# TUMFTM/global_racetrajectory_optimization

Measured on NVIDIA H100. Metric: min-curv QPs/sec (N=1000 closed track, batched), higher is better.
Workload: dtype f64

## Files before the change

### global_racetrajectory_optimization_b200/csrc/mincurv_ipm.cu

```cuda
#include <cstdio>
#include <cstdlib>
#include "mincurv_ops.cuh"

namespace mc {

constexpr unsigned FULL = 0xffffffffu;
constexpr int IP_THREADS = 64;
constexpr int SUB = 8;
constexpr int VBP = 12;
constexpr int FROW = 34;
constexpr int HB_SLOTS = 2;
constexpr int HO_SLOTS = 2;
constexpr int LROW = 33;
#ifndef MC_LT_SLOTS
#define MC_LT_SLOTS 3
#endif
constexpr int LT_SLOTS = MC_LT_SLOTS;
constexpr int GT_SLOTS = 6 - LT_SLOTS;
constexpr int RING_UNITS = LT_SLOTS + GT_SLOTS;
constexpr int QDEPTH = 16;
constexpr int LT_UNIT_DOUBLES = SUB * LROW;
constexpr int GT_UNIT_DOUBLES = SUB * FROW;
constexpr unsigned HB_UNIT_BYTES = SUB * HB_PITCH * sizeof(double);

__device__ __forceinline__ void dmma(double (&c)[2], double a, double b) {
    asm volatile("mma.sync.aligned.m8n8k4.row.col.f64.f64.f64.f64 {%0,%1}, {%2}, {%3}, {%0,%1};\n"
                 : "+d"(c[0]), "+d"(c[1]) : "d"(a), "d"(b));
}

__device__ __forceinline__ uint32_t smem_u32(const void *p) { return (uint32_t)__cvta_generic_to_shared(p); }
__device__ __forceinline__ void mbar_init(uint64_t *bar, unsigned count) {
    asm volatile("mbarrier.init.shared::cta.b64 [%0], %1;" ::"r"(smem_u32(bar)), "r"(count) : "memory");
}
__device__ __forceinline__ void mbar_expect_tx(uint64_t *bar, unsigned bytes) {
    asm volatile("mbarrier.arrive.expect_tx.shared::cta.b64 _, [%0], %1;" ::"r"(smem_u32(bar)), "r"(bytes) : "memory");
}
__device__ __forceinline__ void mbar_arrive(uint64_t *bar) {
    asm volatile("mbarrier.arrive.shared::cta.b64 _, [%0];" ::"r"(smem_u32(bar)) : "memory");
}
#ifndef MC_WAIT_MODE
#define MC_WAIT_MODE 1
#endif
#ifndef MC_RELAXED_BACKOFF_NS
#define MC_RELAXED_BACKOFF_NS 250
#endif

__device__ __forceinline__ void mbar_wait(uint64_t *bar, unsigned parity) {
#if MC_WAIT_MODE == 0
    asm volatile("{\n .reg .pred p;\n WAIT_%=:\n mbarrier.try_wait.parity.shared::cta.b64 p, [%0], %1, 0x989680;\n"
                 " @p bra DONE_%=;\n bra WAIT_%=;\n DONE_%=:\n}" ::"r"(smem_u32(bar)), "r"(parity) : "memory");
#else
    asm volatile("{\n .reg .pred p;\n WAIT_%=:\n mbarrier.test_wait.parity.shared::cta.b64 p, [%0], %1;\n"
                 " @p bra DONE_%=;\n bra WAIT_%=;\n DONE_%=:\n}" ::"r"(smem_u32(bar)), "r"(parity) : "memory");
#endif
}
__device__ __forceinline__ void mbar_wait_relaxed(uint64_t *bar, unsigned parity) {
#ifndef MC_RELAXED_SPIN_NS
    unsigned ok = 0;
    for (;;) {
        asm volatile("{\n .reg .pred p;\n mbarrier.try_wait.parity.shared::cta.b64 p, [%1], %2, 0x989680;\n selp.u32 %0, 1, 0, p;\n}"
                     : "=r"(ok) : "r"(smem_u32(bar)), "r"(parity) : "memory");
        if (ok) break;
        __nanosleep(MC_RELAXED_BACKOFF_NS);
// ... 61 lines not shown
#define SEG_BEGIN() do { } while (0)
#define SEG(slot) do { } while (0)
#define PROF_T0(name) do { } while (0)
#define PROF_ADD(slot, t0) do { } while (0)
#define PROF_ADD1(slot, t0) do { } while (0)
#endif

__device__ __forceinline__ double fast_rcp(double d) {
    double x;
    asm("rcp.approx.ftz.f64 %0, %1;" : "=d"(x) : "d"(d));
    double e = fma(-d, x, 1.0);
    x = fma(x, e, x);
    e = fma(-d, x, 1.0);
    return fma(x, e, x);
}

struct Handoff {
    double vb[32 * VBP];
    double l11[64];
    double w[8], y[8];
};

struct IpShared {
    union {
        struct {
            double hb[HB_SLOTS][SUB * HB_PITCH];
            Handoff ho[HO_SLOTS];
            double gb[32 * VBP];
        } f;
        struct {
            double lt[LT_SLOTS][LT_UNIT_DOUBLES];
            double gt[GT_SLOTS][GT_UNIT_DOUBLES];
            double q[QDEPTH * SUB];
        } sw;
        double win[hband_win_doubles(IP_THREADS)];
    } u;
    union {
        double Ss[32 * 33];
        double sfrag[20 * 32];
    } s;
    double wS[32], gs[32], part[2][32];
    double red[32];
    uint64_t hb_full[HB_SLOTS], ho_full[HO_SLOTS], ho_empty[HO_SLOTS], ring_full[RING_UNITS];
    unsigned ring_phase[2];
    int prog[4];
    int flag;
    int next;
    int resumed;
};

struct Factor {
    const double *HB;
    const double *DD;
    double *LT, *GT;
    int NA;
};

__device__ __forceinline__ Factor make_factor(double *slab, const Layout &L, int n, const double *HB) {
    double *LT = slab + L.o_tiles;
    return {HB, vec(slab, L, V_DD), LT, LT + (size_t)L.np * LROW, n - 32};
}

__device__ __forceinline__ int lt_slot(int c, int m) { return LROW * c + ((m + 3 * c - 1) & 31); }
__device__ __forceinline__ double lt_entry(const double *unit, int c, int m) {
    return (c < m && m <= c + 32) ? unit[lt_slot(c, m)] : 0.0;
}

__device__ __forceinline__ int blk(int I, int J) { return (I * (I + 1)) / 2 + J; }

__device__ __noinline__ bool factor_chain(IpShared &sh, const double *__restrict__ HBp, const double *__restrict__ DD, double *__restrict__ LTp, const int NA, const double *__restrict__ g, unsigned tick) {
    const int lane = threadIdx.x & 31;
    const int gq = lane >> 2, q = lane & 3;
    const int nunits = (NA + SUB - 1) / SUB;
    const uint64_t pol = l2_evict_normal_policy();
    double W[10][2];
#pragma unroll
    for (int b = 0; b < 10; ++b) { W[b][0] = 0.0; W[b][1] = 0.0; }
    double gv = (lane < NA) ? g[lane] : 0.0;
    double gcur = (32 + lane < NA) ? g[32 + lane] : 0.0;
    double gnext = (64 + lane < NA) ? g[64 + lane] : 0.0;
    double ddcur = (lane < NA) ? DD[lane] : 0.0;
    double ddnext = (32 + lane < NA) ? DD[32 + lane] : 0.0;
    bool ok = true;
    if (lane == 0) {
        mbar_expect_tx(&sh.hb_full[tick % HB_SLOTS], HB_UNIT_BYTES);
        tma_load_1d(sh.u.f.hb[tick % HB_SLOTS], HBp, HB_UNIT_BYTES, &sh.hb_full[tick % HB_SLOTS], pol);
    }
    SEG_BEGIN();
    for (int t = 0; t < nunits; ++t) {
        const unsigned ht = tick + t, hs = ht % HB_SLOTS, ls = ht % HO_SLOTS;
        const int k0 = t * SUB;
        SEG(8);
        if (t > 0 && (t & 3) == 0) {
            gcur = gnext;
            ddcur = ddnext;
            const int idx = k0 + 64 + lane, idd = k0 + 32 + lane;
            gnext = (idx < NA) ? g[idx] : 0.0;
            ddnext = (idd < NA) ? DD[idd] : 0.0;
        }
        if (lane == 0 && t + 1 < nunits) {
            const unsigned h2 = (ht + 1) % HB_SLOTS;
            mbar_expect_tx(&sh.hb_full[h2], HB_UNIT_BYTES);
            tma_load_1d(sh.u.f.hb[h2], HBp + (size_t)(t + 1) * SUB * HB_PITCH, HB_UNIT_BYTES, &sh.hb_full[h2], pol);
        }
        PROF_T0(tw1);
        if (ht >= (unsigned)HO_SLOTS) mbar_wait(&sh.ho_empty[ls], ((ht / HO_SLOTS) - 1u) & 1u);
        PROF_ADD(PROF_W0_WAIT_HO_EMPTY, tw1);
        Handoff &ho = sh.u.f.ho[ls];
        SEG(9);
#pragma unroll
        for (int I = 0; I < 4; ++I)
            *reinterpret_cast<double2 *>(&ho.vb[(8 * I + gq) * VBP + 2 * q]) = make_double2(W[blk(I, 0)][0], W[blk(I, 0)][1]);
        __syncwarp();
// ... 57 lines not shown
            ho.w[lane] = wsave;
            ho.y[lane] = ysave;
        }
        __syncwarp();
        {
            const int jq = lane & 7;
            double q8[8];
#pragma unroll
            for (int m = 0; m < 8; ++m) {
                double sacc = (m == jq) ? 1.0 : 0.0;
#pragma unroll
                for (int i = 0; i < m; ++i) sacc = fma(-ho.l11[m * 8 + i], q8[i], sacc);
                q8[m] = sacc;
            }
            if (lane < 8) {
                double *ltq = ltp + 36 * lane - 1;
#pragma unroll
                for (int m = 1; m < 8; ++m)
                    if (m > lane) st_stream(ltq + m, q8[m]);
                st_stream(ltp + lane * LROW + 32, wsave);
            }
        }
        double af[4][2], bf[4][2];
#pragma unroll
        for (int ks = 0; ks < 2; ++ks) {
            const double dk = __shfl_sync(FULL, dsave, 4 * ks + q);
#pragma unroll
            for (int I = 0; I < 4; ++I) {
                bf[I][ks] = ho.vb[(8 * I + gq) * VBP + 4 * ks + q];
                af[I][ks] = bf[I][ks] * dk;
            }
        }
#pragma unroll
        for (int I = 0; I < 4; ++I)
#pragma unroll
            for (int J = 0; J <= I; ++J) {
                double c[2] = {0.0, 0.0};
                if (I < 3) { c[0] = W[blk(I + 1, J + 1)][0]; c[1] = W[blk(I + 1, J + 1)][1]; }
                dmma(c, af[I][0], bf[J][0]);
                dmma(c, af[I][1], bf[J][1]);
                W[blk(I, J)][0] = c[0]; W[blk(I, J)][1] = c[1];
            }
        {
            const double up = __shfl_sync(FULL, gv, (lane + 8) & 31), en = __shfl_sync(FULL, gv2, (lane - 24) & 31);
            gv = (lane < 24) ? up : en;
        }
        __syncwarp();
        SEG(12);
        if (lane == 0) mbar_arrive(&sh.ho_full[ls]);
    }
    return ok;
}

__device__ __noinline__ void factor_fill(IpShared &sh, const double *__restrict__ HBp, double *__restrict__ GTp, const int NA, const double *__restrict__ g, unsigned tick) {
    const int lane = threadIdx.x & 31;
    const int gq = lane >> 2, q = lane & 3;
    const int nunits = (NA + SUB - 1) / SUB;
    double G[4][4][2];
#pragma unroll
    for (int I = 0; I < 4; ++I)
#pragma unroll
        for (int J = 0; J < 4; ++J) { G[I][J][0] = 0.0; G[I][J][1] = 0.0; }
    double gsacc = 0.0;
    double *gb = sh.u.f.gb;
    for (int t = 0; t < nunits; ++t) {
        const unsigned ht = tick + t, ls = ht % HO_SLOTS;
        const int k0 = t * SUB;
#pragma unroll
        for (int I = 0; I < 4; ++I)
            *reinterpret_cast<double2 *>(&gb[(8 * I + gq) * VBP + 2 * q]) = make_double2(G[I][0][0], G[I][0][1]);
        __syncwarp();
        double gp[8];
#pragma unroll
        for (int j = 0; j < 8; j += 2) {
            const double2 uu = *reinterpret_cast<const double2 *>(&gb[lane * VBP + j]);
            gp[j] = uu.x; gp[j + 1] = uu.y;
        }
        const bool hasY = (k0 < 32) || (k0 + SUB - 1 >= NA - 32);
        if (hasY) {
#pragma unroll
            for (int j = 0; j < 8; ++j) {
                const int k = k0 + j;
                double yv = 0.0;
                if (k < NA) {
                    if (k <= lane) yv = HBp[(size_t)(NA + lane) * HB_PITCH + (k + 32 - lane)];
                    else if (k >= NA + lane - 32) yv = HBp[(size_t)k * HB_PITCH + (NA + lane - k)];
                }
                gp[j] = yv - gp[j];
            }
        } else {
#pragma unroll
            for (int j = 0; j < 8; ++j) gp[j] = -gp[j];
        }
        __syncwarp();
        PROF_T0(tw2);
        mbar_wait_relaxed(&sh.ho_full[ls], (ht / HO_SLOTS) & 1u);
        PROF_ADD1(PROF_W1_WAIT_HO_FULL, tw2);
        const Handoff &ho = sh.u.f.ho[ls];
#pragma unroll
        for (int m = 0; m < 7; ++m)
#pragma unroll
            for (int j = m + 1; j < 8; ++j) gp[j] = fma(-gp[m], ho.l11[j * 8 + m], gp[j]);
        double *gtp = GTp + (size_t)k0 * FROW;
#pragma unroll
        for (int j = 0; j < 8; ++j) {
            st_stream(gtp + j * FROW + lane, gp[j]);
            gsacc = fma(gp[j], ho.w[j] * ho.y[j], gsacc);
        }
        if (lane < 8) {
            const double w = ho.w[lane];
            *reinterpret_cast<double2 *>(gtp + lane * FROW + 32) = make_double2(w * ho.y[lane], w);
        }
#pragma unroll
        for (int j = 0; j < 8; j += 2) *reinterpret_cast<double2 *>(&gb[lane * VBP + j]) = make_double2(gp[j], gp[j + 1]);
        __syncwarp();
        PROF_T0(tw3);
        double af[4][2], bf[4][2], wq[2];
#pragma unroll
        for (int ks = 0; ks < 2; ++ks) {
            wq[ks] = ho.w[4 * ks + q];
#pragma unroll
            for (int I = 0; I < 4; ++I) {
                af[I][ks] = gb[(8 * I + gq) * VBP + 4 * ks + q];
                bf[I][ks] = ho.vb[(8 * I + gq) * VBP + 4 * ks + q];
            }
        }
#pragma unroll
        for (int I = 0; I < 4; ++I)
#pragma unroll
            for (int J = 0; J < 4; ++J) {
                double c[2] = {0.0, 0.0};
                if (J < 3) { c[0] = G[I][J + 1][0]; c[1] = G[I][J + 1][1]; }
                dmma(c, af[I][0], bf[J][0]);
                dmma(c, af[I][1], bf[J][1]);
                G[I][J][0] = c[0]; G[I][J][1] = c[1];
            }
#pragma unroll
        for (int I = 0; I < 4; ++I) {
            double c2[4][2];
#pragma unroll
            for (int J = 0; J <= I; ++J) {
                const double2 cc = *reinterpret_cast<const double2 *>(&sh.s.sfrag[(blk(I, J) * 32 + lane) * 2]);
                c2[J][0] = cc.x; c2[J][1] = cc.y;
            }
#pragma unroll
            for (int ks = 0; ks < 2; ++ks) {
                const double a = af[I][ks] * wq[ks];
#pragma unroll
                for (int J = 0; J <= I; ++J) dmma(c2[J], a, af[J][ks]);
            }
#pragma unroll
            for (int J = 0; J <= I; ++J)
                *reinterpret_cast<double2 *>(&sh.s.sfrag[(blk(I, J) * 32 + lane) * 2]) = make_double2(c2[J][0], c2[J][1]);
        }
        __syncwarp();
        PROF_ADD1(PROF_W1_UPDATE, tw3);
        if (lane == 0) mbar_arrive(&sh.ho_empty[ls]);
    }
    sh.gs[lane] = g[NA + lane] - gsacc;
}

__device__ __forceinline__ unsigned factor_units(int n) { return (unsigned)((n - 32 + SUB - 1) / SUB); }
__device__ __noinline__ bool factor(IpShared &sh, double *slab, const Layout &L, int n, const double *HB, const double *g, unsigned tick) {
    const Factor F = make_factor(slab, L, n, HB);
    const int NA = F.NA;
    const int warp = threadIdx.x >> 5, lane = threadIdx.x & 31;
    for (int e = threadIdx.x; e < 20 * 32; e += IP_THREADS) sh.s.sfrag[e] = 0.0;
    fence_proxy_async();
    __syncthreads();
    PROF_T0(tc0);
    if (warp == 0) {
        if (!factor_chain(sh, F.HB, F.DD, F.LT, NA, g, tick)) sh.flag = 1;
        PROF_ADD(PROF_CHAIN, tc0);
    } else {
        factor_fill(sh, F.HB, F.GT, NA, g, tick);
        PROF_ADD1(PROF_FILL, tc0);
    }
    PROF_T0(tc1);
    double sf[20];
    if (warp == 1) {
#pragma unroll
        for (int e = 0; e < 20; ++e) sf[e] = sh.s.sfrag[((e >> 1) * 32 + lane) * 2 + (e & 1)];
    }
    double sv[16];
#pragma unroll
    for (int i = 0; i < 16; ++i) {
        const int e = threadIdx.x + i * IP_THREADS;
        const int r = e >> 5, c = e & 31;
        const int lo = min(r, c), dist = abs(r - c);
        sv[i] = F.HB[(size_t)(NA + lo) * HB_PITCH + dist];
        if (r == c) sv[i] += F.DD[NA + r];
    }
    __syncthreads();
#pragma unroll
    for (int i = 0; i < 16; ++i) {
        const int e = threadIdx.x + i * IP_THREADS;
        sh.s.Ss[(e >> 5) * 33 + (e & 31)] = sv[i];
    }
    __syncthreads();
    if (warp == 1) {
        const int gq = lane >> 2, q = lane & 3;
#pragma unroll
        for (int I = 0; I < 4; ++I)
#pragma unroll
            for (int J = 0; J <= I; ++J) {
                const int bi = (I * (I + 1)) / 2 + J;
#pragma unroll
                for (int e = 0; e < 2; ++e) {
                    const int r = 8 * I + gq, c = 8 * J + 2 * q + e;
                    sh.s.Ss[r * 33 + c] -= sf[2 * bi + e];
                    if (I != J) sh.s.Ss[c * 33 + r] -= sf[2 * bi + e];
                }
            }
        __syncwarp();
        bool ok = true;
#pragma unroll 1
        for (int k = 0; k < 32; ++k) {
            const double d = sh.s.Ss[k * 33 + k];
            if (!(d > 0.0)) ok = false;
            const double w = fast_rcp(d);
            const double l = sh.s.Ss[lane * 33 + k] * w;
            if (lane > k) {
#pragma unroll 4
                for (int c = k + 1; c < 32; ++c) sh.s.Ss[lane * 33 + c] = fma(-l, sh.s.Ss[k * 33 + c], sh.s.Ss[lane * 33 + c]);
                sh.s.Ss[lane * 33 + k] = l;
            }
            if (lane == k) sh.wS[k] = w;
            __syncwarp();
// ... 13 lines not shown
    unsigned phase;
    uint64_t pol;
    const double *rows;
    int nunits, last;
    bool down;
    int sl, sn;
    __device__ RingT(IpShared &s, double *b, const double *r, int nu, bool dn)
        : sh(s), buf(b), phase(s.ring_phase[WHO]), pol(l2_evict_first_policy()), rows(r), nunits(nu), last(nu - 1), down(dn), sl(0), sn(AHEAD) {}
    __device__ __forceinline__ int unit(int i) const { return down ? last - i : i; }
    __device__ __forceinline__ void issue(int u, int slot) {
        const unsigned bytes = (unsigned)(UNIT_DOUBLES * sizeof(double));
        mbar_expect_tx(&sh.ring_full[BASE + slot], bytes);
        tma_load_1d(buf + slot * UNIT_DOUBLES, rows + (size_t)u * UNIT_DOUBLES, bytes, &sh.ring_full[BASE + slot], pol);
    }
    __device__ __forceinline__ void prime() {
        if ((threadIdx.x & 31) == 0) for (int i = 0; i < AHEAD && i < nunits; ++i) issue(unit(i), i);
    }
    __device__ __forceinline__ const double *wait() {
#ifdef MC_PROFILE
        const long long tw = clock64();
#endif
        mbar_wait(&sh.ring_full[BASE + sl], (phase >> sl) & 1u);
#ifdef MC_PROFILE
        if (blockIdx.x == 0 && (threadIdx.x & 31) == 0) atomicAdd(&g_prof[PROF_RING_WAIT_W0 + WHO], (unsigned long long)(clock64() - tw));
#endif
        phase ^= 1u << sl;
        return buf + sl * UNIT_DOUBLES;
    }
    __device__ __forceinline__ void refill(int i) { if (i + AHEAD < nunits) issue(down ? unit(i) - AHEAD : unit(i) + AHEAD, sn); }
    __device__ __forceinline__ void next() {
        sl = (sl == SLOTS - 1) ? 0 : sl + 1;
        sn = (sn == SLOTS - 1) ? 0 : sn + 1;
    }
    __device__ __forceinline__ void close() { sh.ring_phase[WHO] = phase; }
};
using LtRing = RingT<LT_SLOTS, 0, LT_UNIT_DOUBLES, 0>;
using GtRing = RingT<GT_SLOTS, LT_SLOTS, GT_UNIT_DOUBLES, 1>;

__device__ __forceinline__ void prog_publish(int *p, int v) { asm volatile("st.release.cta.shared.s32 [%0], %1;" ::"r"(smem_u32(p)), "r"(v) : "memory"); }
__device__ __forceinline__ int prog_read(const int *p) {
    int v;
    asm volatile("ld.acquire.cta.shared.s32 %0, [%1];" : "=r"(v) : "r"(smem_u32(p)) : "memory");
    return v;
}
template <bool BACKOFF = false>
__device__ __forceinline__ void prog_wait(IpShared &sh, const int *p, int need) {
    for (int spin = 0; spin < (1 << 18); ++spin) {
        if (prog_read(p) >= need) return;
        if (BACKOFF) __nanosleep(MC_RELAXED_BACKOFF_NS);
    }
    sh.flag = 1;
}

__device__ __noinline__ void sweep_forward(IpShared &sh, double *__restrict__ LTp, double *__restrict__ GTp, const int NA, const double *__restrict__ g) {
    const int lane = threadIdx.x & 31;
    const int gq = lane >> 2, q = lane & 3;
    const int nunits = (NA + SUB - 1) / SUB;
    LtRing R(sh, &sh.u.sw.lt[0][0], LTp, nunits, false);
    R.prime();
    double acc[4];
#pragma unroll
    for (int I = 0; I < 4; ++I) acc[I] = (8 * I + gq < NA) ? g[8 * I + gq] : 0.0;
    double gcur = (32 + lane < NA) ? g[32 + lane] : 0.0;
    double gnext = (64 + lane < NA) ? g[64 + lane] : 0.0;
    for (int u = 0; u < nunits; ++u, R.next()) {
        const int k0 = u * SUB;
        if (u > 0 && (u & 3) == 0) {
            gcur = gnext;
            const int idx = k0 + 64 + lane;
            gnext = (idx < NA) ? g[idx] : 0.0;
        }
        if ((u & 7) == 0 && u >= 8) prog_wait(sh, &sh.prog[1], u - 8);
        const double *lt = R.wait();
        const double ge = __shfl_sync(FULL, gcur, ((u & 3) << 3) + gq);
        double a[5][2];
#pragma unroll
        for (int I = 0; I < 5; ++I) {
            a[I][0] = lt_entry(lt, q, 8 * I + gq);
            a[I][1] = lt_entry(lt, 4 + q, 8 * I + gq);
        }
        const double wl = lt[gq * LROW + 32];
        const double b0 = __shfl_sync(FULL, acc[0], 4 * q), b1 = __shfl_sync(FULL, acc[0], 16 + 4 * q);
        double y0[2] = {acc[0], acc[0]}, y1[2] = {0.0, 0.0};
        dmma(y0, a[0][0], b0);
        dmma(y1, a[0][1], b1);
        const double y = y0[0] + y1[0];
        const double n0 = -__shfl_sync(FULL, y, 4 * q), n1 = -__shfl_sync(FULL, y, 16 + 4 * q);
        double nw[4];
#pragma unroll
        for (int I = 0; I < 4; ++I) {
            const double c = (I < 3) ? acc[I + 1] : ge;
            double c0[2] = {c, c}, c1[2] = {0.0, 0.0};
            dmma(c0, a[I + 1][0], n0);
            dmma(c1, a[I + 1][1], n1);
            nw[I] = c0[0] + c1[0];
        }
        if (q == 0) {
            const bool in = (k0 + gq < NA);
            const double z = in ? y * wl : 0.0;
            sh.u.sw.q[(u & (QDEPTH - 1)) * SUB + gq] = z;
            if (in) GTp[(size_t)(k0 + gq) * FROW + 32] = z;
        }
#pragma unroll
        for (int I = 0; I < 4; ++I) acc[I] = nw[I];
        __syncwarp();
        if (lane == 0) { prog_publish(&sh.prog[0], u + 1); R.refill(u); }
    }
    R.close();
    fence_proxy_async();
}

__device__ __noinline__ void sweep_sep_rhs(IpShared &sh, double *__restrict__ GTp, const int NA, const double *__restrict__ g) {
    const int lane = threadIdx.x & 31;
    const int nunits = (NA + SUB - 1) / SUB;
    GtRing R(sh, &sh.u.sw.gt[0][0], GTp, nunits, false);
    R.prime();
    double s0 = 0.0, s1 = 0.0;
    const double gsl = g[NA + lane];
    for (int u = 0; u < nunits; ++u, R.next()) {
        const double *gt = R.wait() + lane;
        prog_wait<true>(sh, &sh.prog[0], u + 1);
        const double *zq = &sh.u.sw.q[(u & (QDEPTH - 1)) * SUB];
#pragma unroll
        for (int s2 = 0; s2 < SUB; s2 += 2) {
            s0 = fma(gt[s2 * FROW], zq[s2], s0);
            s1 = fma(gt[(s2 + 1) * FROW], zq[s2 + 1], s1);
        }
        __syncwarp();
        if (lane == 0) { prog_publish(&sh.prog[1], u + 1); R.refill(u); }
    }
    R.close();
    sh.gs[lane] = gsl - (s0 + s1);
}

__device__ __noinline__ void sweep_sep_solve(IpShared &sh, double *__restrict__ GTp, const int NA, double *__restrict__ x) {
    const int lane = threadIdx.x & 31;
    const int nunits = (NA + SUB - 1) / SUB;
    GtRing R(sh, &sh.u.sw.gt[0][0], GTp, nunits, true);
    R.prime();
    double a = sh.gs[lane];
#pragma unroll 4
    for (int k = 0; k < 32; ++k) {
        const double yk = __shfl_sync(FULL, a, k);
        const double l = (lane > k) ? sh.s.Ss[lane * 33 + k] : 0.0;
        a = fma(-l, yk, a);
    }
    a *= sh.wS[lane];
#pragma unroll 4
    for (int k = 31; k >= 0; --k) {
        const double xk = __shfl_sync(FULL, a, k);
        const double l = (lane < k) ? sh.s.Ss[k * 33 + lane] : 0.0;
        a = fma(-l, xk, a);
    }
    x[NA + lane] = a;
    const int kl = lane & 7, qr = lane >> 3;
    double xq[8];
#pragma unroll
    for (int i = 0; i < 8; ++i) xq[i] = __shfl_sync(FULL, a, 8 * qr + i);
    for (int i = 0; i < nunits; ++i, R.next()) {
        const int k = R.unit(i) * SUB + kl;
        if ((i & 7) == 0 && i >= 8) prog_wait<true>(sh, &sh.prog[2], i - 8);
        const double *gt = R.wait() + kl * FROW;
        const double2 zw = *reinterpret_cast<const double2 *>(&gt[32]);
        double c0 = 0.0, c1 = 0.0;
#pragma unroll
        for (int e = 0; e < 8; e += 2) {
            const double2 gg = *reinterpret_cast<const double2 *>(&gt[8 * qr + e]);
            c0 = fma(gg.x, xq[e], c0);
            c1 = fma(gg.y, xq[e + 1], c1);
        }
        double c = c0 + c1;
        c += __shfl_xor_sync(FULL, c, 8);
        c += __shfl_xor_sync(FULL, c, 16);
        if (qr == 0) sh.u.sw.q[(i & (QDEPTH - 1)) * SUB + kl] = (k < NA) ? fma(-c, zw.y, zw.x) : 0.0;
        __syncwarp();
        if (lane == 0) { prog_publish(&sh.prog[3], i + 1); R.refill(i); }
    }
    R.close();
}

__device__ __noinline__ void sweep_backward(IpShared &sh, double *__restrict__ LTp, const int NA, double *__restrict__ x) {
    const int lane = threadIdx.x & 31;
    const int gq = lane >> 2, q = lane & 3;
    const int nunits = (NA + SUB - 1) / SUB;
    LtRing R(sh, &sh.u.sw.lt[0][0], LTp, nunits, true);
    R.prime();
    double nbx[8];
#pragma unroll
    for (int i = 0; i < 8; ++i) nbx[i] = 0.0;
    for (int i = 0; i < nunits; ++i, R.next()) {
        const int k0 = R.unit(i) * SUB;
        const double *lt = R.wait();
        double a[10];
#pragma unroll
        for (int c = 0; c < 10; ++c) a[c] = lt_entry(lt, gq, 4 * c + q);
        double c0[2] = {0.0, 0.0}, c1[2] = {0.0, 0.0};
#pragma unroll
        for (int e = 2; e < 8; e += 2) {
            dmma(c0, a[2 + e], nbx[e]);
            dmma(c1, a[3 + e], nbx[e + 1]);
        }
        dmma(c0, a[2], nbx[0]);
        dmma(c1, a[3], nbx[1]);
        prog_wait(sh, &sh.prog[3], i + 1);
        const double t1 = sh.u.sw.q[(i & (QDEPTH - 1)) * SUB + gq];
        const double uu = t1 + (c0[0] + c1[0]);
        const double u0 = __shfl_sync(FULL, uu, 4 * q), u1 = __shfl_sync(FULL, uu, 16 + 4 * q);
        double d0[2] = {uu, uu}, d1[2] = {0.0, 0.0};
        dmma(d0, a[0], u0);
        dmma(d1, a[1], u1);
        const double x1 = d0[0] + d1[0];
        if (q == 0 && k0 + gq < NA) x[k0 + gq] = x1;
#pragma unroll
        for (int e = 7; e >= 2; --e) nbx[e] = nbx[e - 2];
        nbx[0] = -__shfl_sync(FULL, x1, 4 * q);
        nbx[1] = -__shfl_sync(FULL, x1, 16 + 4 * q);
        __syncwarp();
        if (lane == 0) { prog_publish(&sh.prog[2], i + 1); R.refill(i); }
    }
    R.close();
}

__device__ __noinline__ void solve(IpShared &sh, double *slab, const Layout &L, int n, const double *g, double *x, bool fused) {
    const Factor F = make_factor(slab, L, n, nullptr);
    const int warp = threadIdx.x >> 5;
    if (threadIdx.x < 4) sh.prog[threadIdx.x] = 0;
    fence_proxy_async();
    __syncthreads();
    if (!fused) {
        PROF_T0(t0);
        if (warp == 0) sweep_forward(sh, F.LT, F.GT, F.NA, g);
        else sweep_sep_rhs(sh, F.GT, F.NA, g);
        __syncthreads();
        PROF_ADD1(PROF_FWD_SWEEPS, t0);
    }
    PROF_T0(t3);
    if (warp == 1) sweep_sep_solve(sh, F.GT, F.NA, x);
    else sweep_backward(sh, F.LT, F.NA, x);
    __syncthreads();
    PROF_ADD1(PROF_BWD_SWEEPS, t3);
}

__device__ void band_matvec(const double *__restrict__ HB, const double *__restrict__ v, double *__restrict__ out, int n) {
    for (int i = threadIdx.x; i < n; i += IP_THREADS) {
        const double *row = HB + (size_t)i * HB_PITCH;
        double s = row[0] * v[i];
        int j = i;
        for (int k = 1; k <= HBW; ++k) {
            j = (j + 1 == n) ? 0 : j + 1;
            s = fma(row[k], v[j], s);
        }
        j = i;
        for (int k = 1; k <= HBW; ++k) {
            j = (j == 0) ? n - 1 : j - 1;
            s = fma(HB[(size_t)j * HB_PITCH + k], v[j], s);
        }
        out[i] = s;
    }
}

__device__ __forceinline__ IpShared &ip_init_shared() {
    extern __shared__ __align__(16) unsigned char smem_raw[];
    IpShared &sh = *reinterpret_cast<IpShared *>(smem_raw);
    if (threadIdx.x == 0) {
        for (int i = 0; i < HB_SLOTS; ++i) mbar_init(&sh.hb_full[i], 1);
        for (int i = 0; i < HO_SLOTS; ++i) { mbar_init(&sh.ho_full[i], 1); mbar_init(&sh.ho_empty[i], 1); }
        for (int i = 0; i < RING_UNITS; ++i) mbar_init(&sh.ring_full[i], 1);
        sh.ring_phase[0] = 0; sh.ring_phase[1] = 0;
        asm volatile("fence.mbarrier_init.release.cluster;" ::: "memory");
    }
    __syncthreads();
    return sh;
}

__device__ __forceinline__ int next_instance(IpShared &sh, int *work_counter) {
    __syncthreads();
    if (threadIdx.x == 0) sh.next = atomicAdd(work_counter, 1);
    __syncthreads();
    return sh.next;
}

constexpr int V_PARK = V_VV;
enum ParkSlot {
    PARK_MU = 0, PARK_MU0 = 1, PARK_RDTOL = 2, PARK_IT = 3,
    PARK_TRACE = 8,
    PARK_MU_HIST = 16,
    PARK_LIST = 64
};
constexpr int PARK_BUCKETS = 24;
enum SchedSlot { SCHED_WORK = 0, SCHED_COUNT = 8, SCHED_TAKEN = 40 };
// ... 26 lines not shown
__device__ __forceinline__ int next_work(IpShared &sh, int *sched, double *ws, const Layout &L, int B) {
    __syncthreads();
    if (threadIdx.x == 0) {
        int b = B, resumed = 0;
        if (ld_relaxed(&sched[SCHED_WORK]) < B) b = atomicAdd(&sched[SCHED_WORK], 1);
        if (b >= B) {
            b = B;
            for (int k = PARK_BUCKETS - 1; k >= 0 && !resumed; --k) {
                int t = ld_relaxed(&sched[SCHED_TAKEN + k]);
                while (t < ld_relaxed(&sched[SCHED_COUNT + k])) {
                    const int seen = atomicCAS(&sched[SCHED_TAKEN + k], t, t + 1);
                    if (seen != t) { t = seen; continue; }
                    const int *e = &park_list(ws, L, t)[k];
                    int v = 0;
                    for (int spin = 0; spin < (1 << 24) && (v = ld_relaxed(e)) == 0; ++spin) __nanosleep(64);
                    __threadfence();
                    if (v > 0) { b = v - 1; resumed = 1; }
                    break;
                }
            }
        }
        sh.next = b;
        sh.resumed = resumed;
    }
    __syncthreads();
    return sh.next;
}

#ifdef MC_TAIL_TRACE
__device__ __forceinline__ double trace_clock() {
    unsigned long long t;
    asm volatile("mov.u64 %0, %%globaltimer;" : "=l"(t));
    return __longlong_as_double((long long)t);
}
#endif

template <bool ADD_ITERS>
__device__ __forceinline__ void write_instance(double *aout, int n, int n_max, const double *AL, int b, int result, int it,
                                               int32_t *status, int32_t *iters_out) {
    __syncthreads();
    for (int i = threadIdx.x; i < n_max; i += IP_THREADS) aout[i] = (i < n) ? AL[i] : 0.0;
    if (threadIdx.x == 0) {
        status[b] = result;
        if (iters_out) iters_out[b] = ADD_ITERS ? iters_out[b] + it : it;
    }
}

__device__ __forceinline__ double affine_step(double r) { return (r > 1.0) ? 1.0 / r : 1.0; }
__device__ __forceinline__ double centring(double c00, double c01, double c10, double c11, double ap, double ad, double mu, double m) {
    const double sigma = (c00 + ad * c01 + ap * c10 + ap * ad * c11) / m / mu;
    return sigma * sigma * sigma * mu;
}
__device__ __forceinline__ double damped_step(double eta, double r) { return (eta < r) ? eta / r : 1.0; }

__global__ void __launch_bounds__(IP_THREADS, 8)
mincurv_pdip_kernel(int B, int n_max, const int32_t *__restrict__ n_pts, double *__restrict__ ws, Layout L,
                    PdipParams prm, int slice, double *__restrict__ alpha_out, int32_t *__restrict__ status,
                    int32_t *__restrict__ iters_out, int *__restrict__ sched) {
#ifdef MC_DEBUG_SM_LIMIT
    {
        unsigned smid;
        asm volatile("mov.u32 %0, %%smid;" : "=r"(smid));
        if (smid >= MC_DEBUG_SM_LIMIT) return;
    }
#endif
    IpShared &sh = ip_init_shared();
    unsigned tick = 0;
    for (int b; (b = next_work(sh, sched, ws, L, B)) < B;) {
        const bool resume = sh.resumed;
        const int n = n_pts ? n_pts[b] : n_max;
        double *aout = alpha_out + (size_t)b * n_max;
        if (!resume && status[b] != 0) {
            for (int i = threadIdx.x; i < n_max; i += IP_THREADS) aout[i] = 0.0;
            if (iters_out && threadIdx.x == 0) iters_out[b] = 0;
            continue;
        }
        PROF_T0(tq0);
#ifdef MC_TAIL_TRACE
        if (threadIdx.x == 0) {
            double *PK = park_slots(ws, L, b);
            if (!resume) {
                unsigned smid;
                asm volatile("mov.u32 %0, %%smid;" : "=r"(smid));
                PK[PARK_TRACE + 2] = 0.0; PK[PARK_TRACE + 3] = 0.0; PK[PARK_TRACE + 5] = smid;
                PK[PARK_TRACE + 6] = 0.0; PK[PARK_TRACE + 7] = 0.0;
            }
            PK[PARK_TRACE + (resume ? 2 : 0)] = trace_clock();
        }
#endif
        double *slab = ws + (size_t)b * L.stride;
        const double *HB = ws + (size_t)*band_owner(slab, L) * L.stride + L.o_hb;
        const double *__restrict__ LB = vec(slab, L, V_LB), *__restrict__ UB = vec(slab, L, V_UB), *__restrict__ F = vec(slab, L, V_F);
        double *__restrict__ AL = vec(slab, L, V_ALPHA), *__restrict__ LU = vec(slab, L, V_LU), *__restrict__ LL = vec(slab, L, V_LL), *__restrict__ RD = vec(slab, L, V_RD);
        double *__restrict__ RHS = vec(slab, L, V_RHS), *__restrict__ DX = vec(slab, L, V_DX), *__restrict__ DD = vec(slab, L, V_DD);
        double *__restrict__ TU = vec(slab, L, V_DLU), *__restrict__ TL = vec(slab, L, V_DLL), *__restrict__ SU = vec(slab, L, V_SU), *__restrict__ SL = vec(slab, L, V_SL);
        double *__restrict__ ISU = vec(slab, L, V_ISU), *__restrict__ ISL = vec(slab, L, V_ISL);
        double *G0 = vec(slab, L, V_T0);
        if (threadIdx.x == 0) sh.flag = 0;
        double mu0, rd_tol, mu;
        int it;
        if (resume) {
            const double *PK = park_slots(ws, L, b);
            mu = PK[PARK_MU]; mu0 = PK[PARK_MU0]; rd_tol = PK[PARK_RDTOL]; it = (int)PK[PARK_IT];
        } else {
            for (int i = threadIdx.x; i < n; i += IP_THREADS) AL[i] = 0.5 * (LB[i] + UB[i]);
            __syncthreads();
            band_matvec(HB, AL, G0, n);
            __syncthreads();
            double gmax = 0.0, fmaxv = 0.0;
#pragma unroll 1
            for (int i = threadIdx.x; i < n; i += IP_THREADS) {
                const double gi = G0[i] + F[i];
                G0[i] = gi;
                gmax = fmax(gmax, fabs(gi));
                fmaxv = fmax(fmaxv, fabs(F[i]));
            }
            gmax = block_reduce<1>(gmax, sh.red);
            fmaxv = block_reduce<1>(fmaxv, sh.red);
            const double lam0 = prm.lam0_rel * gmax + 1e-300;
            double musum = 0.0;
#pragma unroll 1
            for (int i = threadIdx.x; i < n; i += IP_THREADS) {
                const double gi = G0[i];
                const double lu = fmax(-gi, 0.0) + lam0, ll = fmax(gi, 0.0) + lam0;
                const double rd = gi + lu - ll;
                LU[i] = lu; LL[i] = ll;
                RD[i] = rd;
                const double a = AL[i];
                const double su = UB[i] - a, sl = a - LB[i];
                const double isu = 1.0 / su, isl = 1.0 / sl;
                SU[i] = su; SL[i] = sl;
                ISU[i] = isu; ISL[i] = isl;
                DD[i] = lu * isu + ll * isl; RHS[i] = -rd + lu - ll;
                musum += su * lu + sl * ll;
            }
            musum = block_reduce<0>(musum, sh.red);
            mu0 = musum / (2.0 * n);
            rd_tol = prm.rd_rel * (fmaxv + gmax) + 1e-300;
            mu = mu0;
            it = 0;
        }
        int result = -1;
        const int it_end = (slice > 0 && !resume) ? min(slice, prm.max_iter) : prm.max_iter;

        constexpr int VG = 4, VS = VG * IP_THREADS;
        for (; it < it_end; ++it) {
            PROF_T0(tf0);
            const bool fok = factor(sh, slab, L, n, HB, RHS, tick);
            tick += factor_units(n);
            if (!fok) { result = 3; break; }
            PROF_ADD(PROF_FACTOR, tf0);
            PROF_T0(ts0);
            solve(sh, slab, L, n, RHS, DX, true);
            PROF_ADD(PROF_SOLVE_PRED, ts0);
            PROF_T0(tv2);
            double rp = 0.0, rdl = 0.0, c00 = 0.0, c01 = 0.0, c10 = 0.0, c11 = 0.0;
#pragma unroll 1
            for (int i0 = threadIdx.x; i0 < n; i0 += VS) {
                double su[VG], sl[VG], lu[VG], ll[VG], dx[VG], isu[VG], isl[VG];
#pragma unroll
                for (int k = 0; k < VG; ++k) {
                    const int i = min(i0 + k * IP_THREADS, n - 1);
                    su[k] = SU[i]; sl[k] = SL[i]; lu[k] = LU[i]; ll[k] = LL[i]; dx[k] = DX[i]; isu[k] = ISU[i]; isl[k] = ISL[i];
                }
#pragma unroll
                for (int k = 0; k < VG; ++k) {
                    if (i0 + k * IP_THREADS < n) {
                        const double p = dx[k] * isu[k], m = dx[k] * isl[k];
                        rp = fmax(rp, fmax(p, -m));
                        rdl = fmax(rdl, fmax(1.0 - p, 1.0 + m));
                        const double dlu = lu[k] * (p - 1.0), dll = -ll[k] * (1.0 + m);
                        c00 += su[k] * lu[k] + sl[k] * ll[k];
                        c01 += su[k] * dlu + sl[k] * dll;
                        c10 += dx[k] * (ll[k] - lu[k]);
                        c11 += dx[k] * (dll - dlu);
                    }
                }
            }
            rp = block_reduce<1>(rp, sh.red);
            rdl = block_reduce<1>(rdl, sh.red);
            double ap = affine_step(rp), ad = affine_step(rdl);
            c00 = block_reduce<0>(c00, sh.red); c01 = block_reduce<0>(c01, sh.red);
            c10 = block_reduce<0>(c10, sh.red); c11 = block_reduce<0>(c11, sh.red);
            const double smu = centring(c00, c01, c10, c11, ap, ad, mu, 2.0 * n);
            PROF_ADD(PROF_AFFINE, tv2);
            PROF_T0(tv3);
#pragma unroll 1
            for (int i0 = threadIdx.x; i0 < n; i0 += VS) {
                double su[VG], sl[VG], lu[VG], ll[VG], dx[VG], isu[VG], isl[VG], rd[VG];
#pragma unroll
                for (int k = 0; k < VG; ++k) {
                    const int i = min(i0 + k * IP_THREADS, n - 1);
                    su[k] = SU[i]; sl[k] = SL[i]; lu[k] = LU[i]; ll[k] = LL[i]; dx[k] = DX[i]; isu[k] = ISU[i]; isl[k] = ISL[i]; rd[k] = RD[i];
                }
#pragma unroll
                for (int k = 0; k < VG; ++k) {
                    const int i = i0 + k * IP_THREADS;
                    if (i < n) {
                        const double dlu = lu[k] * (dx[k] * isu[k] - 1.0), dll = -ll[k] * (1.0 + dx[k] * isl[k]);
                        const double tu = smu - su[k] * lu[k] + dx[k] * dlu;
                        const double tl = smu - sl[k] * ll[k] - dx[k] * dll;
                        TU[i] = tu; TL[i] = tl;
                        RHS[i] = -rd[k] - tu * isu[k] + tl * isl[k];
                    }
                }
            }
            __syncthreads();
            PROF_ADD(PROF_CORR_RHS, tv3);
            PROF_T0(ts1);
            solve(sh, slab, L, n, RHS, DX, false);
            PROF_ADD(PROF_SOLVE_CORR, ts1);
            PROF_T0(tv4);
            rp = 0.0; rdl = 0.0;
#pragma unroll 1
            for (int i0 = threadIdx.x; i0 < n; i0 += VS) {
                double lu[VG], ll[VG], dx[VG], isu[VG], isl[VG], tu[VG], tl[VG];
#pragma unroll
                for (int k = 0; k < VG; ++k) {
                    const int i = min(i0 + k * IP_THREADS, n - 1);
                    lu[k] = LU[i]; ll[k] = LL[i]; dx[k] = DX[i]; isu[k] = ISU[i]; isl[k] = ISL[i]; tu[k] = TU[i]; tl[k] = TL[i];
                }
#pragma unroll
                for (int k = 0; k < VG; ++k) {
                    if (i0 + k * IP_THREADS < n) {
                        const double dlu = (tu[k] + lu[k] * dx[k]) * isu[k], dll = (tl[k] - ll[k] * dx[k]) * isl[k];
                        rp = fmax(rp, fmax(dx[k] * isu[k], -dx[k] * isl[k]));
                        rdl = fmax(rdl, fmax(-dlu / lu[k], -dll / ll[k]));
                    }
                }
            }
            rp = block_reduce<1>(rp, sh.red);
            rdl = block_reduce<1>(rdl, sh.red);
            ap = damped_step(prm.eta, rp);
            ad = damped_step(prm.eta, rdl);
            PROF_ADD(PROF_STEPLEN, tv4);
            PROF_T0(tv5);
            double musum2 = 0.0, rdmax = 0.0, dxmax = 0.0, amax = 0.0;
            constexpr int VG2 = 2, VS2 = VG2 * IP_THREADS;
#pragma unroll 1
            for (int i0 = threadIdx.x; i0 < n; i0 += VS2) {
                double su[VG2], sl[VG2], lu[VG2], ll[VG2], dx[VG2], isu[VG2], isl[VG2], tu[VG2], tl[VG2], al[VG2], rd[VG2], rh[VG2], dd[VG2];
#pragma unroll
                for (int k = 0; k < VG2; ++k) {
                    const int i = min(i0 + k * IP_THREADS, n - 1);
                    su[k] = SU[i]; sl[k] = SL[i]; lu[k] = LU[i]; ll[k] = LL[i]; dx[k] = DX[i]; isu[k] = ISU[i]; isl[k] = ISL[i];
                    tu[k] = TU[i]; tl[k] = TL[i]; al[k] = AL[i]; rd[k] = RD[i]; rh[k] = RHS[i]; dd[k] = DD[i];
                }
#pragma unroll
                for (int k = 0; k < VG2; ++k) {
                    const int i = i0 + k * IP_THREADS;
                    if (i < n) {
                        const double dlu = (tu[k] + lu[k] * dx[k]) * isu[k], dll = (tl[k] - ll[k] * dx[k]) * isl[k];
                        const double an = al[k] + ap * dx[k], lun = lu[k] + ad * dlu, lln = ll[k] + ad * dll;
                        const double sun = su[k] - ap * dx[k], sln = sl[k] + ap * dx[k];
                        const double rdn = rd[k] + ap * (rh[k] - dd[k] * dx[k]) + ad * (dlu - dll);
                        const double isun = 1.0 / sun, isln = 1.0 / sln;
                        AL[i] = an; LU[i] = lun; LL[i] = lln; RD[i] = rdn; SU[i] = sun; SL[i] = sln;
                        ISU[i] = isun; ISL[i] = isln;
                        DD[i] = lun * isun + lln * isln; RHS[i] = -rdn + lun - lln;
                        musum2 += sun * lun + sln * lln;
                        rdmax = fmax(rdmax, fabs(rdn));
                        dxmax = fmax(dxmax, fabs(dx[k]));
                        amax = fmax(amax, fabs(an));
                    }
                }
            }
            if (threadIdx.x == 0) park_slots(ws, L, b)[PARK_MU] = mu;
            mu = block_reduce<0>(musum2, sh.red) / (2.0 * n);
            rdmax = block_reduce<1>(rdmax, sh.red);
            PROF_ADD(PROF_UPDATE, tv5);
#ifdef MC_TAIL_TRACE
            if (threadIdx.x == 0 && it < PARK_LIST - PARK_MU_HIST) {
                park_slots(ws, L, b)[PARK_MU_HIST + it] = mu;
                park_slots(ws, L, b)[PARK_MU0] = mu0;
            }
#endif
            bool settled = true;
            if (prm.dx_rel > 0.0 && mu <= prm.mu_rel * mu0) {
                dxmax = block_reduce<1>(dxmax, sh.red);
                amax = block_reduce<1>(amax, sh.red);
                settled = ap * dxmax <= prm.dx_rel * fmax(amax, 0.01);
            }
            if (mu <= prm.mu_rel * mu0 && rdmax <= rd_tol && settled) { result = 0; ++it; break; }
            if (mu <= 1e-4 * prm.mu_rel * mu0) { result = (rdmax <= 1e3 * rd_tol) ? 0 : 2; ++it; break; }
        }
        if (result < 0 && it < prm.max_iter) {
            if (threadIdx.x == 0) {
                double *PK = park_slots(ws, L, b);
                const double mu_prev = PK[PARK_MU];
                PK[PARK_MU] = mu; PK[PARK_MU0] = mu0; PK[PARK_RDTOL] = rd_tol; PK[PARK_IT] = it;
#ifdef MC_TAIL_TRACE
                PK[PARK_TRACE + 1] = trace_clock();
                PK[PARK_TRACE + 6] = it;
                PK[PARK_TRACE + 7] = park_bucket(mu, mu_prev, prm.mu_rel * mu0, prm.max_iter - it, n, n);
#endif
                park(sched, ws, L, b, park_bucket(mu, mu_prev, prm.mu_rel * mu0, prm.max_iter - it, n, n_max));
            }
            continue;
        }
        if (result < 0) result = 2;
        write_instance<false>(aout, n, n_max, AL, b, result, it, status, iters_out);
#ifdef MC_TAIL_TRACE
        if (threadIdx.x == 0) {
            double *PK = park_slots(ws, L, b);
            PK[PARK_TRACE + (resume ? 3 : 1)] = trace_clock();
            PK[PARK_TRACE + 4] = it;
        }
#endif
        PROF_ADD(PROF_TOTAL, tq0);
#ifdef MC_PROFILE
        if (blockIdx.x == 0 && threadIdx.x == 0) { atomicAdd(&g_prof[PROF_NQP], 1ull); atomicAdd(&g_prof[PROF_ITERS], (unsigned long long)it); }
// ... 323 lines not shown
```

### global_racetrajectory_optimization_b200/csrc/mincurv_ws.cuh

```cuda
#pragma once
#include "common.cuh"

namespace mc {

enum Vec : int {
    V_H = 0, V_DIAG, V_DFW, V_DBW, V_LFW, V_INVD, V_TII, V_RHOP, V_RHOM,
    V_PX, V_PY, V_NX, V_NY, V_MX, V_MY, V_XP, V_YP, V_SX, V_SY, V_KREF,
    V_LB, V_UB, V_F,
    V_T0, V_T1, V_T2, V_T3, V_T4, V_T5,
    V_ALPHA, V_LU, V_LL, V_RD, V_RHS, V_DX, V_DD, V_DLU, V_DLL, V_SU, V_SL,
    V_ISU, V_ISL, V_HBSRC,
    V_S3, V_S4, V_L3, V_L4, V_KL, V_WK, V_EDX, V_T3K, V_T4K, V_VV,
    V_IH,
    NUM_VEC
};

struct Layout {
    int n_max;
    int np;
    size_t o_zb, o_hb, o_tiles, stride;
};

__host__ __device__ inline Layout make_layout(int n_max) {
    Layout L;
    L.n_max = n_max;
    L.np = ((n_max + 31) / 32) * 32 + 64;
    size_t o = (size_t)NUM_VEC * L.np;
    L.o_zb = o;
    o += (size_t)n_max * ZB_PITCH;
    L.o_hb = o;
    o += (size_t)L.np * HB_PITCH;
    L.o_tiles = o;
    o += (size_t)L.np * 67;
    L.stride = (o + 15) & ~(size_t)15;
    return L;
}

constexpr int SCHED_INTS = 64;

struct PdipParams {
    int max_iter;
    double mu_rel;
    double rd_rel;
    double eta;
    double dx_rel;
    double lam0_rel;
};

__device__ __forceinline__ double *vec(double *slab, const Layout &L, int v) { return slab + (size_t)v * L.np; }

__device__ __forceinline__ int32_t *band_owner(double *slab, const Layout &L) { return reinterpret_cast<int32_t *>(vec(slab, L, V_HBSRC)); }

}
```

Before: 63650.

## Recompute slack inverses and corrector terms instead of storing them; split Z from GT tiles

Removes the stored ISU/ISL/TU/TL vectors from the interior-point loop. Slack reciprocals and corrector terms are now recomputed from SU/SL and a separately kept affine step (DXA), which cuts global memory reads and writes per iteration. The GT tile row narrows from 34 to 33 doubles by moving the z value into its own Z vector, and the separator solve prefetches that value. The cost is extra divides and arithmetic per element, and Z now sits after the GT region in the tiles area, which changes the workspace layout.

After: 70220 (median of 6 runs). +10.3%, better.

```diff
diff --git a/global_racetrajectory_optimization_b200/csrc/mincurv_ipm.cu b/global_racetrajectory_optimization_b200/csrc/mincurv_ipm.cu
--- a/global_racetrajectory_optimization_b200/csrc/mincurv_ipm.cu
+++ b/global_racetrajectory_optimization_b200/csrc/mincurv_ipm.cu
@@ -8,7 +8,7 @@
 constexpr int IP_THREADS = 64;
 constexpr int SUB = 8;
 constexpr int VBP = 12;
-constexpr int FROW = 34;
+constexpr int FROW = 33;
 constexpr int HB_SLOTS = 2;
 constexpr int HO_SLOTS = 2;
 constexpr int LROW = 33;
@@ -176,13 +176,13 @@
 struct Factor {
     const double *HB;
     const double *DD;
-    double *LT, *GT;
+    double *LT, *GT, *Z;
     int NA;
 };
 
 __device__ __forceinline__ Factor make_factor(double *slab, const Layout &L, int n, const double *HB) {
-    double *LT = slab + L.o_tiles;
-    return {HB, vec(slab, L, V_DD), LT, LT + (size_t)L.np * LROW, n - 32};
+    double *LT = slab + L.o_tiles, *GT = LT + (size_t)L.np * LROW;
+    return {HB, vec(slab, L, V_DD), LT, GT, GT + (size_t)L.np * FROW, n - 32};
 }
 
 __device__ __forceinline__ int lt_slot(int c, int m) { return LROW * c + ((m + 3 * c - 1) & 31); }
@@ -346,7 +346,7 @@
     return ok;
 }
 
-__device__ __noinline__ void factor_fill(IpShared &sh, const double *__restrict__ HBp, double *__restrict__ GTp, const int NA, const double *__restrict__ g, unsigned tick) {
+__device__ __noinline__ void factor_fill(IpShared &sh, const double *__restrict__ HBp, double *__restrict__ GTp, double *__restrict__ Zp, const int NA, const double *__restrict__ g, unsigned tick) {
     const int lane = threadIdx.x & 31;
     const int gq = lane >> 2, q = lane & 3;
     const int nunits = (NA + SUB - 1) / SUB;
@@ -403,7 +403,8 @@
         }
         if (lane < 8) {
             const double w = ho.w[lane];
-            *reinterpret_cast<double2 *>(gtp + lane * FROW + 32) = make_double2(w * ho.y[lane], w);
+            st_stream(gtp + lane * FROW + 32, w);
+            Zp[k0 + lane] = w * ho.y[lane];
         }
 #pragma unroll
         for (int j = 0; j < 8; j += 2) *reinterpret_cast<double2 *>(&gb[lane * VBP + j]) = make_double2(gp[j], gp[j + 1]);
@@ -467,7 +468,7 @@
         if (!factor_chain(sh, F.HB, F.DD, F.LT, NA, g, tick)) sh.flag = 1;
         PROF_ADD(PROF_CHAIN, tc0);
     } else {
-        factor_fill(sh, F.HB, F.GT, NA, g, tick);
+        factor_fill(sh, F.HB, F.GT, F.Z, NA, g, tick);
         PROF_ADD1(PROF_FILL, tc0);
     }
     PROF_T0(tc1);
@@ -587,7 +588,7 @@
     sh.flag = 1;
 }
 
-__device__ __noinline__ void sweep_forward(IpShared &sh, double *__restrict__ LTp, double *__restrict__ GTp, const int NA, const double *__restrict__ g) {
+__device__ __noinline__ void sweep_forward(IpShared &sh, double *__restrict__ LTp, double *__restrict__ Zp, const int NA, const double *__restrict__ g) {
     const int lane = threadIdx.x & 31;
     const int gq = lane >> 2, q = lane & 3;
     const int nunits = (NA + SUB - 1) / SUB;
@@ -634,7 +635,7 @@
             const bool in = (k0 + gq < NA);
             const double z = in ? y * wl : 0.0;
             sh.u.sw.q[(u & (QDEPTH - 1)) * SUB + gq] = z;
-            if (in) GTp[(size_t)(k0 + gq) * FROW + 32] = z;
+            if (in) Zp[k0 + gq] = z;
         }
 #pragma unroll
         for (int I = 0; I < 4; ++I) acc[I] = nw[I];
@@ -668,7 +669,7 @@
     sh.gs[lane] = gsl - (s0 + s1);
 }
 
-__device__ __noinline__ void sweep_sep_solve(IpShared &sh, double *__restrict__ GTp, const int NA, double *__restrict__ x) {
+__device__ __noinline__ void sweep_sep_solve(IpShared &sh, double *__restrict__ GTp, const double *Zp, const int NA, double *__restrict__ x) {
     const int lane = threadIdx.x & 31;
     const int nunits = (NA + SUB - 1) / SUB;
     GtRing R(sh, &sh.u.sw.gt[0][0], GTp, nunits, true);
@@ -692,22 +693,24 @@
     double xq[8];
 #pragma unroll
     for (int i = 0; i < 8; ++i) xq[i] = __shfl_sync(FULL, a, 8 * qr + i);
+    double znext = 0.0;
+    if (nunits > 0 && R.unit(0) * SUB + kl < NA) znext = Zp[R.unit(0) * SUB + kl];
     for (int i = 0; i < nunits; ++i, R.next()) {
         const int k = R.unit(i) * SUB + kl;
+        const double z = znext;
+        if (i + 1 < nunits && R.unit(i + 1) * SUB + kl < NA) znext = Zp[R.unit(i + 1) * SUB + kl];
         if ((i & 7) == 0 && i >= 8) prog_wait<true>(sh, &sh.prog[2], i - 8);
         const double *gt = R.wait() + kl * FROW;
-        const double2 zw = *reinterpret_cast<const double2 *>(&gt[32]);
         double c0 = 0.0, c1 = 0.0;
 #pragma unroll
         for (int e = 0; e < 8; e += 2) {
-            const double2 gg = *reinterpret_cast<const double2 *>(&gt[8 * qr + e]);
-            c0 = fma(gg.x, xq[e], c0);
-            c1 = fma(gg.y, xq[e + 1], c1);
+            c0 = fma(gt[8 * qr + e], xq[e], c0);
+            c1 = fma(gt[8 * qr + e + 1], xq[e + 1], c1);
         }
         double c = c0 + c1;
         c += __shfl_xor_sync(FULL, c, 8);
         c += __shfl_xor_sync(FULL, c, 16);
-        if (qr == 0) sh.u.sw.q[(i & (QDEPTH - 1)) * SUB + kl] = (k < NA) ? fma(-c, zw.y, zw.x) : 0.0;
+        if (qr == 0) sh.u.sw.q[(i & (QDEPTH - 1)) * SUB + kl] = (k < NA) ? fma(-c, gt[32], z) : 0.0;
         __syncwarp();
         if (lane == 0) { prog_publish(&sh.prog[3], i + 1); R.refill(i); }
     }
@@ -764,13 +767,13 @@
     __syncthreads();
     if (!fused) {
         PROF_T0(t0);
-        if (warp == 0) sweep_forward(sh, F.LT, F.GT, F.NA, g);
+        if (warp == 0) sweep_forward(sh, F.LT, F.Z, F.NA, g);
         else sweep_sep_rhs(sh, F.GT, F.NA, g);
         __syncthreads();
         PROF_ADD1(PROF_FWD_SWEEPS, t0);
     }
     PROF_T0(t3);
-    if (warp == 1) sweep_sep_solve(sh, F.GT, F.NA, x);
+    if (warp == 1) sweep_sep_solve(sh, F.GT, F.Z, F.NA, x);
     else sweep_backward(sh, F.LT, F.NA, x);
     __syncthreads();
     PROF_ADD1(PROF_BWD_SWEEPS, t3);
@@ -903,6 +906,12 @@
     return sigma * sigma * sigma * mu;
 }
 __device__ __forceinline__ double damped_step(double eta, double r) { return (eta < r) ? eta / r : 1.0; }
+__device__ __forceinline__ void corrector_terms(double smu, double su, double sl, double lu, double ll, double dx, double isu,
+                                                double isl, double &tu, double &tl) {
+    const double dlu = lu * (dx * isu - 1.0), dll = -ll * (1.0 + dx * isl);
+    tu = smu - su * lu + dx * dlu;
+    tl = smu - sl * ll - dx * dll;
+}
 
 __global__ void __launch_bounds__(IP_THREADS, 8)
 mincurv_pdip_kernel(int B, int n_max, const int32_t *__restrict__ n_pts, double *__restrict__ ws, Layout L,
@@ -943,9 +952,8 @@
         const double *HB = ws + (size_t)*band_owner(slab, L) * L.stride + L.o_hb;
         const double *__restrict__ LB = vec(slab, L, V_LB), *__restrict__ UB = vec(slab, L, V_UB), *__restrict__ F = vec(slab, L, V_F);
         double *__restrict__ AL = vec(slab, L, V_ALPHA), *__restrict__ LU = vec(slab, L, V_LU), *__restrict__ LL = vec(slab, L, V_LL), *__restrict__ RD = vec(slab, L, V_RD);
-        double *__restrict__ RHS = vec(slab, L, V_RHS), *__restrict__ DX = vec(slab, L, V_DX), *__restrict__ DD = vec(slab, L, V_DD);
-        double *__restrict__ TU = vec(slab, L, V_DLU), *__restrict__ TL = vec(slab, L, V_DLL), *__restrict__ SU = vec(slab, L, V_SU), *__restrict__ SL = vec(slab, L, V_SL);
-        double *__restrict__ ISU = vec(slab, L, V_ISU), *__restrict__ ISL = vec(slab, L, V_ISL);
+        double *__restrict__ RHS = vec(slab, L, V_RHS), *__restrict__ DX = vec(slab, L, V_DX), *__restrict__ DXA = vec(slab, L, V_DXA);
+        double *__restrict__ DD = vec(slab, L, V_DD), *__restrict__ SU = vec(slab, L, V_SU), *__restrict__ SL = vec(slab, L, V_SL);
         double *G0 = vec(slab, L, V_T0);
         if (threadIdx.x == 0) sh.flag = 0;
         double mu0, rd_tol, mu;
@@ -981,7 +989,6 @@
                 const double su = UB[i] - a, sl = a - LB[i];
                 const double isu = 1.0 / su, isl = 1.0 / sl;
                 SU[i] = su; SL[i] = sl;
-                ISU[i] = isu; ISL[i] = isl;
                 DD[i] = lu * isu + ll * isl; RHS[i] = -rd + lu - ll;
                 musum += su * lu + sl * ll;
             }
@@ -1002,22 +1009,23 @@
             if (!fok) { result = 3; break; }
             PROF_ADD(PROF_FACTOR, tf0);
             PROF_T0(ts0);
-            solve(sh, slab, L, n, RHS, DX, true);
+            solve(sh, slab, L, n, RHS, DXA, true);
             PROF_ADD(PROF_SOLVE_PRED, ts0);
             PROF_T0(tv2);
             double rp = 0.0, rdl = 0.0, c00 = 0.0, c01 = 0.0, c10 = 0.0, c11 = 0.0;
 #pragma unroll 1
             for (int i0 = threadIdx.x; i0 < n; i0 += VS) {
-                double su[VG], sl[VG], lu[VG], ll[VG], dx[VG], isu[VG], isl[VG];
+                double su[VG], sl[VG], lu[VG], ll[VG], dx[VG];
 #pragma unroll
                 for (int k = 0; k < VG; ++k) {
                     const int i = min(i0 + k * IP_THREADS, n - 1);
-                    su[k] = SU[i]; sl[k] = SL[i]; lu[k] = LU[i]; ll[k] = LL[i]; dx[k] = DX[i]; isu[k] = ISU[i]; isl[k] = ISL[i];
+                    su[k] = SU[i]; sl[k] = SL[i]; lu[k] = LU[i]; ll[k] = LL[i]; dx[k] = DXA[i];
                 }
 #pragma unroll
                 for (int k = 0; k < VG; ++k) {
                     if (i0 + k * IP_THREADS < n) {
-                        const double p = dx[k] * isu[k], m = dx[k] * isl[k];
+                        const double isu = 1.0 / su[k], isl = 1.0 / sl[k];
+                        const double p = dx[k] * isu, m = dx[k] * isl;
                         rp = fmax(rp, fmax(p, -m));
                         rdl = fmax(rdl, fmax(1.0 - p, 1.0 + m));
                         const double dlu = lu[k] * (p - 1.0), dll = -ll[k] * (1.0 + m);
@@ -1038,21 +1046,20 @@
             PROF_T0(tv3);
 #pragma unroll 1
             for (int i0 = threadIdx.x; i0 < n; i0 += VS) {
-                double su[VG], sl[VG], lu[VG], ll[VG], dx[VG], isu[VG], isl[VG], rd[VG];
+                double su[VG], sl[VG], lu[VG], ll[VG], dx[VG], rd[VG];
 #pragma unroll
                 for (int k = 0; k < VG; ++k) {
                     const int i = min(i0 + k * IP_THREADS, n - 1);
-                    su[k] = SU[i]; sl[k] = SL[i]; lu[k] = LU[i]; ll[k] = LL[i]; dx[k] = DX[i]; isu[k] = ISU[i]; isl[k] = ISL[i]; rd[k] = RD[i];
+                    su[k] = SU[i]; sl[k] = SL[i]; lu[k] = LU[i]; ll[k] = LL[i]; dx[k] = DXA[i]; rd[k] = RD[i];
                 }
 #pragma unroll
                 for (int k = 0; k < VG; ++k) {
                     const int i = i0 + k * IP_THREADS;
                     if (i < n) {
-                        const double dlu = lu[k] * (dx[k] * isu[k] - 1.0), dll = -ll[k] * (1.0 + dx[k] * isl[k]);
-                        const double tu = smu - su[k] * lu[k] + dx[k] * dlu;
-                        const double tl = smu - sl[k] * ll[k] - dx[k] * dll;
-                        TU[i] = tu; TL[i] = tl;
-                        RHS[i] = -rd[k] - tu * isu[k] + tl * isl[k];
+                        const double isu = 1.0 / su[k], isl = 1.0 / sl[k];
+                        double tu, tl;
+                        corrector_terms(smu, su[k], sl[k], lu[k], ll[k], dx[k], isu, isl, tu, tl);
+                        RHS[i] = -rd[k] - tu * isu + tl * isl;
                     }
                 }
             }
@@ -1065,17 +1072,20 @@
             rp = 0.0; rdl = 0.0;
 #pragma unroll 1
             for (int i0 = threadIdx.x; i0 < n; i0 += VS) {
-                double lu[VG], ll[VG], dx[VG], isu[VG], isl[VG], tu[VG], tl[VG];
+                double su[VG], sl[VG], lu[VG], ll[VG], dxa[VG], dx[VG];
 #pragma unroll
                 for (int k = 0; k < VG; ++k) {
                     const int i = min(i0 + k * IP_THREADS, n - 1);
-                    lu[k] = LU[i]; ll[k] = LL[i]; dx[k] = DX[i]; isu[k] = ISU[i]; isl[k] = ISL[i]; tu[k] = TU[i]; tl[k] = TL[i];
+                    su[k] = SU[i]; sl[k] = SL[i]; lu[k] = LU[i]; ll[k] = LL[i]; dxa[k] = DXA[i]; dx[k] = DX[i];
                 }
 #pragma unroll
                 for (int k = 0; k < VG; ++k) {
                     if (i0 + k * IP_THREADS < n) {
-                        const double dlu = (tu[k] + lu[k] * dx[k]) * isu[k], dll = (tl[k] - ll[k] * dx[k]) * isl[k];
-                        rp = fmax(rp, fmax(dx[k] * isu[k], -dx[k] * isl[k]));
+                        const double isu = 1.0 / su[k], isl = 1.0 / sl[k];
+                        double tu, tl;
+                        corrector_terms(smu, su[k], sl[k], lu[k], ll[k], dxa[k], isu, isl, tu, tl);
+                        const double dlu = (tu + lu[k] * dx[k]) * isu, dll = (tl - ll[k] * dx[k]) * isl;
+                        rp = fmax(rp, fmax(dx[k] * isu, -dx[k] * isl));
                         rdl = fmax(rdl, fmax(-dlu / lu[k], -dll / ll[k]));
                     }
                 }
@@ -1090,24 +1100,26 @@
             constexpr int VG2 = 2, VS2 = VG2 * IP_THREADS;
 #pragma unroll 1
             for (int i0 = threadIdx.x; i0 < n; i0 += VS2) {
-                double su[VG2], sl[VG2], lu[VG2], ll[VG2], dx[VG2], isu[VG2], isl[VG2], tu[VG2], tl[VG2], al[VG2], rd[VG2], rh[VG2], dd[VG2];
+                double su[VG2], sl[VG2], lu[VG2], ll[VG2], dxa[VG2], dx[VG2], al[VG2], rd[VG2], rh[VG2], dd[VG2];
 #pragma unroll
                 for (int k = 0; k < VG2; ++k) {
                     const int i = min(i0 + k * IP_THREADS, n - 1);
-                    su[k] = SU[i]; sl[k] = SL[i]; lu[k] = LU[i]; ll[k] = LL[i]; dx[k] = DX[i]; isu[k] = ISU[i]; isl[k] = ISL[i];
-                    tu[k] = TU[i]; tl[k] = TL[i]; al[k] = AL[i]; rd[k] = RD[i]; rh[k] = RHS[i]; dd[k] = DD[i];
+                    su[k] = SU[i]; sl[k] = SL[i]; lu[k] = LU[i]; ll[k] = LL[i]; dxa[k] = DXA[i]; dx[k] = DX[i];
+                    al[k] = AL[i]; rd[k] = RD[i]; rh[k] = RHS[i]; dd[k] = DD[i];
                 }
 #pragma unroll
                 for (int k = 0; k < VG2; ++k) {
                     const int i = i0 + k * IP_THREADS;
                     if (i < n) {
-                        const double dlu = (tu[k] + lu[k] * dx[k]) * isu[k], dll = (tl[k] - ll[k] * dx[k]) * isl[k];
+                        const double isu = 1.0 / su[k], isl = 1.0 / sl[k];
+                        double tu, tl;
+                        corrector_terms(smu, su[k], sl[k], lu[k], ll[k], dxa[k], isu, isl, tu, tl);
+                        const double dlu = (tu + lu[k] * dx[k]) * isu, dll = (tl - ll[k] * dx[k]) * isl;
                         const double an = al[k] + ap * dx[k], lun = lu[k] + ad * dlu, lln = ll[k] + ad * dll;
                         const double sun = su[k] - ap * dx[k], sln = sl[k] + ap * dx[k];
                         const double rdn = rd[k] + ap * (rh[k] - dd[k] * dx[k]) + ad * (dlu - dll);
                         const double isun = 1.0 / sun, isln = 1.0 / sln;
                         AL[i] = an; LU[i] = lun; LL[i] = lln; RD[i] = rdn; SU[i] = sun; SL[i] = sln;
-                        ISU[i] = isun; ISL[i] = isln;
                         DD[i] = lun * isun + lln * isln; RHS[i] = -rdn + lun - lln;
                         musum2 += sun * lun + sln * lln;
                         rdmax = fmax(rdmax, fabs(rdn));
diff --git a/global_racetrajectory_optimization_b200/csrc/mincurv_ws.cuh b/global_racetrajectory_optimization_b200/csrc/mincurv_ws.cuh
--- a/global_racetrajectory_optimization_b200/csrc/mincurv_ws.cuh
+++ b/global_racetrajectory_optimization_b200/csrc/mincurv_ws.cuh
@@ -8,7 +8,7 @@
     V_PX, V_PY, V_NX, V_NY, V_MX, V_MY, V_XP, V_YP, V_SX, V_SY, V_KREF,
     V_LB, V_UB, V_F,
     V_T0, V_T1, V_T2, V_T3, V_T4, V_T5,
-    V_ALPHA, V_LU, V_LL, V_RD, V_RHS, V_DX, V_DD, V_DLU, V_DLL, V_SU, V_SL,
+    V_ALPHA, V_LU, V_LL, V_RD, V_RHS, V_DX, V_DXA, V_DD, V_DLU, V_DLL, V_SU, V_SL,
     V_ISU, V_ISL, V_HBSRC,
     V_S3, V_S4, V_L3, V_L4, V_KL, V_WK, V_EDX, V_T3K, V_T4K, V_VV,
     V_IH,
```
